# DanielaCourel/smoothed_particle_hydrodynamics

Measured on AMD Instinct MI355X. Metric: Mparticle-steps/sec (whole node), dam-break, higher is better.
Workload: dtype f32

## Files before the change

smoothed_particle_hydrodynamics_amd/csrc/context.h:

```cpp
#pragma once

#include <stdlib.h>
#include <string.h>

#include <memory>
#include <new>
#include <utility>

#include "cell_build.h"
#include "common_kernels.h"
#include "full_kernels.h"
#include "full_tiled.h"
#include "ref_kernels.h"
#include "sample_kernels.h"
#include "surface_kernels.h"
#include "render_kernels.h"
#include "scene_kernels.h"
#include "tracer_kernels.h"
#include "gauge_kernels.h"
#include "slab_kernels.h"
#include "slab_rccl.h"

namespace {

// ... 127 lines not shown
   int cur = 0;

   DevBuf<uint32_t> key;
   DevBuf<uint32_t> slot;
   DevBuf<uint32_t> perm;
   DevBuf<uint32_t> order;
   DevBuf<uint32_t> cell_count;
   DevBuf<uint32_t> cell_start;
   DevBuf<uint32_t> scan_part;
   DevBuf<uint32_t> big_cells;
   int scan_tiles = 0;

   DevBuf<float> rho;
   DevBuf<float4> velB;
   DevBuf<float> auxc;
   DevBuf<float4> acc;
   DevBuf<int32_t> ncount;
   DevBuf<TileDesc> tile_desc;
   DevBuf<uint32_t> nlist;
   DevBuf<uint32_t> nlist_overflow;
   int fast = 0;
   struct {
      int valid = 0;
      int fast = 0;
      float rho0 = 0.0f, stiffness = 0.0f, kernel3 = 0.0f;
   } terms;
   int uniform_mass = 0;
   int use_tiled = 1;
   int prehashed = 0;
   int no_prehash = 0, no_fused_integrate = 0, no_fused_slab = 0;
// ... 269 lines not shown
   CREATE_TRY(dev_alloc(ctx->big_cells, cap / RANK_BIG + 2));
   CREATE_TRY(hipMemsetAsync(ctx->big_cells, 0, sizeof(uint32_t), ctx->stream));
   CREATE_TRY(hipMemsetAsync(ctx->cell_count, 0, cells_padded * sizeof(uint32_t), ctx->stream));
   CREATE_TRY(hipMemsetAsync(ctx->cell_start, 0, cells_padded * sizeof(uint32_t), ctx->stream));
   CREATE_TRY(dev_alloc(ctx->rho, cap));
   CREATE_TRY(dev_alloc(ctx->acc, cap));
   CREATE_TRY(dev_alloc(ctx->ncount, cap));
   CREATE_TRY(hipMemsetAsync(ctx->rho, 0, cap * sizeof(float), ctx->stream));
   CREATE_TRY(hipMemsetAsync(ctx->acc, 0, cap * sizeof(float4), ctx->stream));
   CREATE_TRY(hipMemsetAsync(ctx->ncount, 0, cap * sizeof(int32_t), ctx->stream));
   CREATE_TRY(dev_alloc(ctx->meta, META_COUNT));
   CREATE_TRY(hipMemsetAsync(ctx->meta, 0, META_COUNT * sizeof(int32_t), ctx->stream));
   if (mode == SPH_HIP_MODE_FULL) {
      CREATE_TRY(dev_alloc(ctx->velB, cap));
      CREATE_TRY(dev_alloc(ctx->auxc, cap));
      CREATE_TRY(dev_alloc(ctx->tile_desc, (size_t)div_up(capacity, TILE_THREADS) + 1));
      ctx->list_cap = NLIST_CAP;
      ctx->list_cap_max = NLIST_CAP_MAX;
      if (const char* v = getenv("SPH_HIP_LIST_CAP")) {
         const int c = atoi(v) / 2 * 2;
         if (c > 0) ctx->list_cap = ctx->list_cap_max = c < 2 ? 2 : (c > NLIST_CAP_MAX ? NLIST_CAP_MAX : c);
      }
      ctx->list_blocks = (size_t)div_up(capacity, TILE_THREADS) + 1;
      const size_t nlist_words = ctx->list_blocks * list_rows(ctx->list_cap) * TILE_THREADS;
      CREATE_TRY(dev_alloc(ctx->nlist, nlist_words));
      CREATE_TRY(hipMemsetAsync(ctx->nlist, 0, nlist_words * sizeof(uint32_t), ctx->stream));
      CREATE_TRY(dev_alloc(ctx->nlist_overflow, (size_t)div_up(capacity, TILE_THREADS) + 1));
      if (const char* v = getenv("SPH_HIP_UNTILED")) ctx->use_tiled = (v[0] == '1') ? 0 : 1;
      CREATE_TRY(pinned_alloc(ctx->tile_feedback, TSTAT_COUNT));
      memset(ctx->tile_feedback, 0, TSTAT_COUNT * sizeof(int));
// ... 56 lines not shown
```

smoothed_particle_hydrodynamics_amd/csrc/full_kernels.h:

```cpp
#pragma once

#include "pair_math.h"

struct RowRanges {
   uint32_t s[9], e[9];
};

__device__ __forceinline__ void row_ranges(const CellGrid& g, const uint32_t* __restrict__ cell_start,
                                           int cx, int cy, int cz, RowRanges& r)
{
   const int x0 = cx - 1 < 0 ? 0 : cx - 1;
   const int x1 = cx + 1 >= g.nx ? g.nx - 1 : cx + 1;
#pragma unroll
   for (int k = 0; k < 9; k++) {
      const int z = cz + k / 3 - 1;
      const int y = cy + k % 3 - 1;
      if (z < 0 || z >= g.nz || y < 0 || y >= g.ny) {
         r.s[k] = 0;
         r.e[k] = 0;
      } else {
         const int row = (z * g.ny + y) * g.nx;
         r.s[k] = cell_start[row + x0];
         r.e[k] = cell_start[row + x1 + 1];
      }
   }
}

template <bool UNIT_SCALE, bool FAST = false>
__device__ __forceinline__ void density_untiled(int p, const float4* __restrict__ posm,
                                                const uint32_t* __restrict__ cell_start,
                                                const float4* __restrict__ velp, const CellGrid& g,
                                                const PairConsts& k, float* __restrict__ rho,
                                                float4* __restrict__ velB, float* __restrict__ auxc,
                                                int32_t* __restrict__ ncount)
{
   const float4 pi = posm[p];
   int cx, cy, cz;
   cell_of(g, pi.x, pi.y, pi.z, cx, cy, cz);
   RowRanges r;
   row_ranges(g, cell_start, cx, cy, cz, r);

   float density = 0.0f;
   int count = 0;
#pragma unroll 1
   for (int row = 0; row < 9; row++) {
      const uint32_t s = row == 0 ? r.s[0] : row == 1 ? r.s[1] : row == 2 ? r.s[2] : row == 3 ? r.s[3]
                       : row == 4 ? r.s[4] : row == 5 ? r.s[5] : row == 6 ? r.s[6] : row == 7 ? r.s[7] : r.s[8];
      const uint32_t e = row == 0 ? r.e[0] : row == 1 ? r.e[1] : row == 2 ? r.e[2] : row == 3 ? r.e[3]
                       : row == 4 ? r.e[4] : row == 5 ? r.e[5] : row == 6 ? r.e[6] : row == 7 ? r.e[7] : r.e[8];
// ... 5 lines not shown
         if (d2 < k.h2) {
            {
               float d = sqrtf(d2);
               if (!UNIT_SCALE) d *= k.sim_scale;
               density_accumulate<UNIT_SCALE>(k, pj.w, d, density);
            }
            count++;
         }
      }
   }
   rho[p] = density;
   const float2 bc = FAST ? neighbor_terms_fast(k, density, pi.w) : neighbor_terms(k, density, pi.w);
   const float4 v = velp[p];
   velB[p] = make_float4(v.x, v.y, v.z, FAST ? bc.y : bc.x);
   auxc[p] = FAST ? bc.x : bc.y;
   ncount[p] = count;
}

template <bool FAST>
__global__ void __launch_bounds__(256)
k_neighbor_terms(const float4* __restrict__ posm, const float4* __restrict__ velp,
                 const float* __restrict__ rho, const int32_t* __restrict__ meta, PairConsts k,
                 float4* __restrict__ velB, float* __restrict__ auxc)
{
   const int p = meta[META_SUM_BEGIN] + blockIdx.x * blockDim.x + threadIdx.x;
   if (p >= meta[META_SUM_END]) return;
   const float2 bc = FAST ? neighbor_terms_fast(k, rho[p], posm[p].w) : neighbor_terms(k, rho[p], posm[p].w);
   const float4 v = velp[p];
   velB[p] = make_float4(v.x, v.y, v.z, FAST ? bc.y : bc.x);
   auxc[p] = FAST ? bc.x : bc.y;
}

template <bool UNIT_SCALE, bool FAST>
__global__ void __launch_bounds__(256)
k_full_density(const float4* __restrict__ posm, const uint32_t* __restrict__ cell_start,
               const float4* __restrict__ velp, const int32_t* __restrict__ meta, CellGrid g,
               PairConsts k, float* __restrict__ rho, float4* __restrict__ velB,
               float* __restrict__ auxc, int32_t* __restrict__ ncount)
{
   const int p = meta[META_SUM_BEGIN] + blockIdx.x * blockDim.x + threadIdx.x;
   if (p >= meta[META_SUM_END]) return;
   density_untiled<UNIT_SCALE, FAST>(p, posm, cell_start, velp, g, k, rho, velB, auxc, ncount);
}

template <bool UNIT_SCALE, bool FAST = false>
__device__ __forceinline__ void accel_untiled(int p, const float4* __restrict__ posm,
                                              const float4* __restrict__ velB,
                                              const float* __restrict__ rho,
                                              const float* __restrict__ auxc,
                                              const uint32_t* __restrict__ cell_start,
                                              const CellGrid& g, const PairConsts& k,
                                              float4* __restrict__ acc,
                                              const int32_t* __restrict__ ncount = nullptr)
{
   const float4 pi = posm[p];
   int cx, cy, cz;
   cell_of(g, pi.x, pi.y, pi.z, cx, cy, cz);
// ... 51 lines not shown
```

smoothed_particle_hydrodynamics_amd/csrc/full_tiled.h:

```cpp
#pragma once

#include "launch_policy.h"
#include "common_kernels.h"
#include "full_kernels.h"
#include "neighbor_lists.h"
#include "slab_kernels.h"

#if defined(SPH_ABLATE) && !defined(SPH_DIAGNOSTIC_BUILD)
#error "SPH_ABLATE is for diagnostic builds only: add -DSPH_DIAGNOSTIC_BUILD (tools/build_variant.sh does)"
#endif

#ifdef SPH_TRIPCOUNT
#ifndef SPH_DIAGNOSTIC_BUILD
#error "SPH_TRIPCOUNT is for diagnostic builds only: add -DSPH_DIAGNOSTIC_BUILD"
#endif
enum {
   TRIP_D_WAVES = 0, TRIP_D_CHUNKS_W, TRIP_D_TEST8_W, TRIP_D_TEST8_L, TRIP_D_SLOTS_L, TRIP_D_POPS_W,
   TRIP_D_POPS_L, TRIP_D_POPLOOPS_W, TRIP_D_SUMTRIPS_W, TRIP_D_SUMSLOTS_W, TRIP_D_LISTED_L, TRIP_D_LANES_L,
   TRIP_A_WAVES = 16, TRIP_A_PTRIPS_W, TRIP_A_CNT_L, TRIP_A_VTRIPS_W, TRIP_A_NV_L, TRIP_A_LANES_L,
   TRIP_COUNT = 32
};
__device__ unsigned long long g_trip[TRIP_COUNT];
struct TripCounters {
   unsigned int v[16];
// ... 30 lines not shown
   }
#define PHASE_COUNT(i) if (threadIdx.x == 0 && blockIdx.x < PHASE_WGS) g_phase[(i) >> 4][blockIdx.x][7] = 1u
#else
#define PHASE_BEGIN()
#define PHASE_MARK(i)
#define PHASE_COUNT(i)
#endif

constexpr int TILE_BATCH = 8;
#define DENSITY_TILE_BYTES 12
#define ACCEL_TILE_BYTES 16
constexpr int DENSITY_BLOCKS = 6 * 256 / TILE_THREADS;
constexpr int ACCEL_BLOCKS = TILE_THREADS == 256 ? 5 : 2;
constexpr int APPEND_POPS = 4;
constexpr int VISC_UNROLL = 4;

typedef float __attribute__((ext_vector_type(2))) f32x2;
typedef float __attribute__((ext_vector_type(4))) f32x4;

__device__ __forceinline__ f32x4 lds_read4(const float* base, int i)
{
   return *reinterpret_cast<const f32x4*>(__builtin_assume_aligned(base + i, 16));
}

struct TileDesc {
   int D[9];
   int B[9];
   int total;
   int pad;
};
// ... 96 lines not shown

__device__ __forceinline__ void tile_desc_load(const TileDesc* __restrict__ desc, int wg, TileDesc& sd)
{
   const int tid = threadIdx.x;
   if (tid < (int)(sizeof(TileDesc) / sizeof(int)))
      reinterpret_cast<int*>(&sd)[tid] = reinterpret_cast<const int*>(&desc[wg])[tid];
   __syncthreads();
}

__device__ __forceinline__ int xcd_workgroup(int block, int nblocks)
{
   const int q = nblocks / 8, r = nblocks % 8, x = block % 8;
   return (x < r ? x * (q + 1) : r * (q + 1) + (x - r) * q) + block / 8;
}

__device__ __forceinline__ void tile_load(const float4* __restrict__ posm, const TileDesc& sd,
                                          const TileLds& L)
{
   const int tid = threadIdx.x;
   const int total = sd.total;
   int B[9], D[9];
#pragma unroll
   for (int k = 0; k < 9; k++) {
      B[k] = sd.B[k];
      D[k] = sd.D[k];
   }
#if defined(SPH_ABLATE) && (SPH_ABLATE == 3 || SPH_ABLATE == 5)
   for (int base = 0; base < 0; base += TILE_BATCH * TILE_THREADS) {
#else
   for (int base = 0; base < total; base += TILE_BATCH * TILE_THREADS) {
#endif
      float4 buf[TILE_BATCH];
#pragma unroll
      for (int r = 0; r < TILE_BATCH; r++) {
         const int idx = min(base + tid + r * TILE_THREADS, total - 1);
         int d = D[0];
#pragma unroll
         for (int k = 1; k < 9; k++) d = (idx >= B[k]) ? D[k] : d;
         buf[r] = posm[idx - d];
      }
#pragma unroll
      for (int r = 0; r < TILE_BATCH; r++) {
         const int idx = base + tid + r * TILE_THREADS;
         if (idx < total) {
            L.x[idx] = buf[r].x;
            L.y[idx] = buf[r].y;
            L.z[idx] = buf[r].z;
         }
      }
   }
   __syncthreads();
}


// ... 46 lines not shown
   m = __builtin_amdgcn_alignbit(m, __float_as_uint(dc.y), 31);
   m = __builtin_amdgcn_alignbit(m, __float_as_uint(dc.x), 31);
   m = __builtin_amdgcn_alignbit(m, __float_as_uint(db.y), 31);
   m = __builtin_amdgcn_alignbit(m, __float_as_uint(db.x), 31);
   m = __builtin_amdgcn_alignbit(m, __float_as_uint(da.y), 31);
   m = __builtin_amdgcn_alignbit(m, __float_as_uint(da.x), 31);
   return m;
}

template <bool UNIT_SCALE, bool UNIFORM_MASS, bool WIDE, bool FAST>
__global__ void __launch_bounds__(TILE_THREADS, WIDE ? (DENSITY_BLOCKS < 4 ? DENSITY_BLOCKS : 4) : DENSITY_BLOCKS)
k_full_density_tiled(const float4* __restrict__ posm, const float4* __restrict__ velp,
                     const uint32_t* __restrict__ cell_start, const int32_t* __restrict__ meta,
                     CellGrid g, PairConsts k, float* __restrict__ rho_out,
                     float4* __restrict__ velB_out, float* __restrict__ auxc_out,
                     int32_t* __restrict__ ncount, const TileDesc* __restrict__ desc,
                     uint32_t* __restrict__ nlist, uint32_t* __restrict__ nlist_overflow,
                     int tile_cap, int32_t* __restrict__ tile_stats,
                     const uint32_t* __restrict__ giveup, int* __restrict__ tile_feedback, int list_cap,
                     double* __restrict__ epart_clear, int inline_giveups)
{
   PHASE_BEGIN();
   if (epart_clear && threadIdx.x < 2) epart_clear[2 * blockIdx.x + threadIdx.x] = 0.0;
   __shared__ TileDesc sd;
   __shared__ int list_overflow;
   TileLds L;
   L.x = tile_lds_dynamic;
   L.y = L.x + (tile_cap + TILE_PAD);
   L.z = L.y + (tile_cap + TILE_PAD);
   if (blockIdx.x == 0 && threadIdx.x < TSTAT_NO_LIST) tile_feedback[threadIdx.x] = tile_stats[threadIdx.x];

   const int begin = meta[META_SUM_BEGIN];
   const int end = meta[META_SUM_END];
   const int tid = threadIdx.x;
   if (inline_giveups && (int)blockIdx.x < tile_stats[TSTAT_GIVEUP_DENSITY]) {
      const int gp = begin + (int)giveup[blockIdx.x] * TILE_THREADS + tid;
      if (gp < end)
         density_untiled<UNIT_SCALE, FAST>(gp, posm, cell_start, velp, g, k, rho_out, velB_out,
                                           auxc_out, ncount);
   }
   const int wgs = tile_stats[TSTAT_BLOCKS];
   const int wg = (int)blockIdx.x < wgs ? xcd_workgroup(blockIdx.x, wgs) : (int)blockIdx.x;
   const int p0 = begin + wg * TILE_THREADS;
   if (p0 >= end) return;
   const int p = p0 + tid;
   const bool live = p < end;
   if (tid == 0) list_overflow = 0;
   float4 pi = make_float4(0.f, 0.f, 0.f, 0.f);
   if (live) pi = posm[p];
   tile_desc_load(desc, wg, sd);
   if (sd.total > tile_cap) {
      if (inline_giveups && tid == 0) nlist_overflow[wg] = LISTS_NONE;
      return;
   }
   char* stage_lane = nullptr;
   const int packed = __builtin_amdgcn_readfirstlane(((sd.total + 31) & ~31) + TILE_PAD);
   const bool staged = (tile_cap + TILE_PAD - packed) * (int)DENSITY_TILE_BYTES >= 16 * TILE_THREADS;
   if (staged) {
      L.y = L.x + packed;
      L.z = L.y + packed;
      stage_lane = reinterpret_cast<char*>(L.z + packed) + 16 * tid;
      list_stage_clear(stage_lane);
   }
   RowRanges r;
#pragma unroll
   for (int kk = 0; kk < 9; kk++) r.s[kk] = r.e[kk] = 0;
   if (live) {
#if !(defined(SPH_ABLATE) && (SPH_ABLATE == 4 || SPH_ABLATE == 5))
      int cx, cy, cz;
      cell_of(g, pi.x, pi.y, pi.z, cx, cy, cz);
      row_ranges(g, cell_start, cx, cy, cz, r);
#endif
   }
   PHASE_MARK(0);
   tile_load(posm, sd, L);
   PHASE_MARK(1);
   const int self_t = p + sd.D[4];
   const f32x2 px = {pi.x, pi.x}, py = {pi.y, pi.y}, pz = {pi.z, pi.z};

   const float h2_screen = k.h2_screen;
   TRIP(TripCounters trips; trips.wave(TRIP_D_WAVES, true); trips.lane(TRIP_D_LANES_L, live ? 1u : 0u);)
   int count = 0;
   ListWriter lw(nlist, wg, list_cap, tid, stage_lane);
   uint32_t pos = list_pos_of(0u);
   auto test_and_append = [&](auto staged_c) {
      constexpr bool STAGED = decltype(staged_c)::value;
#pragma unroll
      for (int kk = 0; kk < 9; kk++) {
         const int D = sd.D[kk];
         const uint32_t kbits = ListEntry<WIDE>::tag(kk);
// ... 150 lines not shown
#endif
   }
   if (!overflowed && kept != count) {
      count = kept;
      lw.pad(count, list_cap);
   }
   TRIP(trips.flush(0, 1u << TRIP_D_TEST8_L | 1u << TRIP_D_SLOTS_L | 1u << TRIP_D_POPS_L | 1u << TRIP_D_LISTED_L |
                       1u << TRIP_D_LANES_L);)
   PHASE_MARK(4);
   if (live) {
      rho_out[p] = density;
      const float2 bc = FAST ? neighbor_terms_fast(k, density, pi.w) : neighbor_terms(k, density, pi.w);
      const float4 v = velp[p];
      velB_out[p] = make_float4(v.x, v.y, v.z, FAST ? bc.y : bc.x);
      auxc_out[p] = FAST ? bc.x : bc.y;
      ncount[p] = count;
   }
   PHASE_MARK(5);
   PHASE_COUNT(15);
}

template <bool UNIT_SCALE, bool UNIFORM_MASS, bool WIDE, bool FAST>
__global__ void __launch_bounds__(TILE_THREADS, 4)
k_full_density_chunked(const float4* __restrict__ posm, const float4* __restrict__ velp,
                       const uint32_t* __restrict__ cell_start, const int32_t* __restrict__ meta,
                       CellGrid g, PairConsts k, float* __restrict__ rho_out,
                       float4* __restrict__ velB_out, float* __restrict__ auxc_out,
                       int32_t* __restrict__ ncount, const TileDesc* __restrict__ desc,
                       uint32_t* __restrict__ nlist, uint32_t* __restrict__ nlist_overflow,
                       int tile_cap, int32_t* __restrict__ tile_stats,
                       const uint32_t* __restrict__ giveup, int list_cap)
{
   __shared__ TileDesc sd;
   __shared__ int list_overflow;
   const int tid = threadIdx.x;
   const bool staged = tile_cap >= 1024;
   const int chunk_cap = staged ? tile_cap - 352 : tile_cap;
   TileLds L;
   L.x = tile_lds_dynamic;
   L.y = L.x + (chunk_cap + TILE_PAD);
   L.z = L.y + (chunk_cap + TILE_PAD);
   char* const stage_lane = reinterpret_cast<char*>(L.z + (chunk_cap + TILE_PAD)) + 16 * tid;
   const int begin = meta[META_SUM_BEGIN], end = meta[META_SUM_END];
   const int n_giveup = tile_stats[TSTAT_GIVEUP_DENSITY];
   for (int gi = blockIdx.x; gi < n_giveup; gi += gridDim.x) {
      const int wg = (int)giveup[gi];
      const int p0 = begin + wg * TILE_THREADS;
      const int p = p0 + tid;
      const bool live = p < end;
      __syncthreads();
      if (tid == 0) list_overflow = 0;
      tile_desc_load(desc, wg, sd);
      if (sd.total + TILE_PAD > (1 << ListEntry<WIDE>::TBITS)) {
         if (live) density_untiled<UNIT_SCALE, FAST>(p, posm, cell_start, velp, g, k, rho_out, velB_out, auxc_out, ncount);
         if (tid == 0) nlist_overflow[wg] = LISTS_NONE;
         continue;
      }
      float4 pi = make_float4(0.f, 0.f, 0.f, 0.f);
      RowRanges r;
#pragma unroll
      for (int kk = 0; kk < 9; kk++) r.s[kk] = r.e[kk] = 0;
      if (live) {
         pi = posm[p];
         int cx, cy, cz;
         cell_of(g, pi.x, pi.y, pi.z, cx, cy, cz);
         row_ranges(g, cell_start, cx, cy, cz, r);
      }
      int cxa, cya, cza, cxb, cyb, czb;
      const float4 pa = posm[p0], pb = posm[min(p0 + TILE_THREADS - 1, end - 1)];
// ... 77 lines not shown
                        } else {
                           count++;
                           if (staged) lw.append<true>(pos, ebase + bit);
                           else lw.append<false>(pos, ebase + bit);
                        }
                     }
                  }
               }
            }
         }
      }
      const bool overflowed = lw.finish(pos, count, list_cap, staged, list_overflow);
      lists_publish(overflowed, list_overflow, tile_stats, nlist_overflow, wg);
      if (live) {
         if (overflowed) {
            density_untiled<UNIT_SCALE, FAST>(p, posm, cell_start, velp, g, k, rho_out, velB_out, auxc_out, ncount);
         } else {
            rho_out[p] = density;
            const float2 bc = FAST ? neighbor_terms_fast(k, density, pi.w) : neighbor_terms(k, density, pi.w);
            const float4 v = velp[p];
            velB_out[p] = make_float4(v.x, v.y, v.z, FAST ? bc.y : bc.x);
            auxc_out[p] = FAST ? bc.x : bc.y;
            ncount[p] = count;
         }
      }
   }
}

struct AccelLds {
   TileDesc desc;
};

__device__ __forceinline__ bool accel_part_has(int part, int p0, const int32_t* __restrict__ meta)
{
   if (part == 0) return true;
   const int ob = meta[META_OWN_BEGIN], oe = meta[META_OWN_END];
   const int lo_end = min(meta[META_BND_LO_END], oe);
// ... 193 lines not shown
            } else {
               accel_pair<UNIT_SCALE>(k, s, dx, dy, dz, dd, UNIFORM_MASS ? pi.w : pj[u].w, vj[u].x, vj[u].y,
                                      vj[u].z, vj[u].w, cj[u], in_range);
            }
         }
      }
   }
   if (FAST) accel_fast_finish(k, s);
   return accel_end<UNIT_SCALE>(k, s);
}

template <bool UNIT_SCALE, bool UNIFORM_MASS, bool WIDE, bool FAST>
__global__ void __launch_bounds__(TILE_THREADS, ACCEL_BLOCKS)
k_full_accel_lists(const float4* __restrict__ posm, const float4* __restrict__ velB,
                   const float* __restrict__ rho, const float* __restrict__ auxc,
                   const int32_t* __restrict__ ncount, const uint32_t* __restrict__ cell_start,
                   const int32_t* __restrict__ meta, CellGrid g, PairConsts k,
                   float4* __restrict__ acc, const TileDesc* __restrict__ desc,
                   const uint32_t* __restrict__ nlist, const uint32_t* __restrict__ nlist_overflow,
                   int tile_cap, const int32_t* __restrict__ tile_stats,
                   const uint32_t* __restrict__ giveup, int part, int list_cap,
                   int* __restrict__ tile_feedback, FusedStep fs, int tile_cap_density)
{
   PHASE_BEGIN();
   __shared__ AccelLds L;
   float4* xyzc = reinterpret_cast<float4*>(tile_lds_dynamic);
   constexpr int BATCH = TILE_BATCH;

   const int begin = meta[META_SUM_BEGIN], end = meta[META_SUM_END];
   const int ob = meta[META_OWN_BEGIN], oe = meta[META_OWN_END];
// ... 2 lines not shown
   const int mapped = accel_part_workgroup(part, blockIdx.x, wgs, begin, meta);
   const int wg = mapped < 0 ? 0 : mapped;
   const int p0 = begin + wg * TILE_THREADS;
   if (blockIdx.x == 0 && tid == 0) {
      tile_feedback[TSTAT_NO_LIST] = tile_stats[TSTAT_NO_LIST];
      if (fs.slab && part == 1) {
         if (fs.left) fs.left->header[1] = fs.msg_capacity;
         if (fs.right) fs.right->header[1] = fs.msg_capacity;
      }
   }
   const bool own = mapped >= 0 && !(p0 >= end || p0 + TILE_THREADS <= ob || p0 >= oe) &&
                    accel_part_has(part, p0, meta);
   const uint32_t gave_up = own ? nlist_overflow[wg] : LISTS_NONE;
   int desc_word = 0;
   if (tid < (int)(sizeof(TileDesc) / sizeof(int))) desc_word = reinterpret_cast<const int*>(&desc[wg])[tid];
   if ((int)blockIdx.x < tile_stats[TSTAT_GIVEUP_ACCEL]) {
      const int g0 = begin + (int)giveup[blockIdx.x] * TILE_THREADS;
      const int gp = g0 + tid;
      const bool mine = gp < end && gp >= ob && gp < oe && accel_part_has(part, g0, meta);
      const int gwg = (int)giveup[blockIdx.x];
      const uint32_t glists = nlist_overflow[gwg];
      if (glists != LISTS_NONE) {
         tile_desc_load(desc, gwg, L.desc);
         if (mine) {
            const int gcnt = ncount[gp];
            const ListReader glr(nlist, gwg, list_cap, tid);
            if (glists == LISTS_SOME && gcnt > 0 && glr.no_list())
               accel_untiled<UNIT_SCALE, FAST>(gp, posm, velB, rho, auxc, cell_start, g, k, acc, ncount);
            else
               acc[gp] = accel_from_lists<UNIT_SCALE, UNIFORM_MASS, WIDE, FAST>(gp, gcnt, glr, L.desc, posm, velB,
// ... 4 lines not shown
         accel_untiled<UNIT_SCALE, FAST>(gp, posm, velB, rho, auxc, cell_start, g, k, acc, ncount);
      }
      if (fs.on && accel_part_has(part, g0, meta)) {
         float4 gx = make_float4(0.f, 0.f, 0.f, 0.f), ga = gx;
         if (mine) {
            gx = posm[gp];
            ga = acc[gp];
         }
         fused_integrate<UNIT_SCALE>(fs, k, g, gp, mine, gx, ga, (int)giveup[blockIdx.x]);
      }
   }
   if (gave_up == LISTS_NONE) return;
   if (tid < (int)(sizeof(TileDesc) / sizeof(int))) reinterpret_cast<int*>(&L.desc)[tid] = desc_word;
   __syncthreads();
   PHASE_MARK(16);
   const int total = L.desc.total;
   if (total > tile_cap || total > tile_cap_density) return;
   int B[9], D[9];
#pragma unroll
   for (int kk = 0; kk < 9; kk++) {
      B[kk] = L.desc.B[kk];
      D[kk] = L.desc.D[kk];
   }
   float4 buf[BATCH];
   float cbuf[BATCH];
#if defined(SPH_ABLATE) && SPH_ABLATE == 23
#pragma unroll
   for (int r = 0; r < BATCH; r++) {
      buf[r] = make_float4(0.f, 0.f, 0.f, 0.f);
      cbuf[r] = 0.f;
   }
   const int filled = 0;
#else
#pragma unroll
   for (int r = 0; r < BATCH; r++) {
      const int idx = min(tid + r * TILE_THREADS, total - 1);
      int d = D[0];
#pragma unroll
      for (int kk = 1; kk < 9; kk++) d = (idx >= B[kk]) ? D[kk] : d;
      buf[r] = posm[idx - d];
      cbuf[r] = auxc[idx - d];
   }
   const int filled = total;
#endif

   const int col = tid;
   const int p = p0 + col;
   const bool live = p < end && p >= ob && p < oe;
   float4 pi = make_float4(0.f, 0.f, 0.f, 0.f);
   float4 vi = pi;
   float rho_i = 0.0f;
   int cnt = 0;
   if (live) {
      pi = posm[p];
      vi = velB[p];
      rho_i = rho[p];
      cnt = ncount[p];
   }

   const ListReader lr(nlist, wg, list_cap, col);
   uint32_t entry[LIST_BLOCK_ENTRIES];
   uint4 next_blk = lr.block(0);

#pragma unroll
   for (int r = 0; r < BATCH; r++) {
      const int idx = tid + r * TILE_THREADS;
      if (idx < filled) xyzc[idx] = make_float4(buf[r].x, buf[r].y, buf[r].z, cbuf[r]);
   }

   AccelState s;
   int first_v = 0;
   bool no_list = false;
   float4 vpre[VISC_UNROLL];
   int tpre[VISC_UNROLL], nvp = 0;
   uint32_t ev[VISC_UNROLL];
   if constexpr (FAST) {
      static_assert(VISC_UNROLL == 4, "list_entries_from takes four entries");
      accel_begin(k, s, pi, vi, rho_i);
      first_v = visc_first(cnt, s.visc_scale);
      const int lcnt = cnt <= list_cap ? cnt : 0;
      const int fv = lcnt > 0 ? first_v : 0;
      const int lb = lcnt > 0 ? (lcnt - 1) >> 3 : 0;
      const int fb = fv >> 3;
      const uint4 blk_a = lr.block(fb), blk_b = lr.block(min(fb + 1, lb));
      if (gave_up == LISTS_SOME && cnt > 0) no_list = next_blk.x == NLIST_NO_LIST;
      nvp = no_list ? 0 : lcnt - fv;
      list_entries_from(blk_a, blk_b, (uint32_t)(fv & 7), ev);
   }

   for (int base = BATCH * TILE_THREADS; base < filled; base += BATCH * TILE_THREADS) {
#pragma unroll
      for (int r = 0; r < BATCH; r++) {
         const int idx = min(base + tid + r * TILE_THREADS, filled - 1);
         int d = D[0];
#pragma unroll
         for (int kk = 1; kk < 9; kk++) d = (idx >= B[kk]) ? D[kk] : d;
         buf[r] = posm[idx - d];
         cbuf[r] = auxc[idx - d];
      }
#pragma unroll
      for (int r = 0; r < BATCH; r++) {
         const int idx = base + tid + r * TILE_THREADS;
         if (idx < filled) xyzc[idx] = make_float4(buf[r].x, buf[r].y, buf[r].z, cbuf[r]);
      }
   }
   if constexpr (FAST) {
#pragma unroll
      for (int u = 0; u < VISC_UNROLL; u++) {
         tpre[u] = ListEntry<WIDE>::tile(ev[u]);
         vpre[u] = make_float4(0.f, 0.f, 0.f, 0.f);
         if (u < nvp) vpre[u] = velB[tpre[u] - ListEntry<WIDE>::shift(L.desc, ev[u])];
      }
   }
   __syncthreads();

   PHASE_MARK(17);
   if constexpr (!FAST) accel_begin(k, s, pi, vi, rho_i);
   const bool in_range = accel_operands_in_range(k);
   if constexpr (!FAST) {
      if (gave_up == LISTS_SOME && cnt > 0) no_list = next_blk.x == NLIST_NO_LIST;
   }
   if (no_list) cnt = 0;
#if defined(SPH_ABLATE) && (SPH_ABLATE == 21 || SPH_ABLATE == 23)
   cnt = 0;
#endif
   const int lastb = cnt > 0 ? (cnt - 1) >> 3 : 0;
   if constexpr (FAST) {
      TRIP(TripCounters trips; trips.wave(TRIP_A_WAVES - 16, true); trips.lane(TRIP_A_CNT_L - 16, (unsigned)cnt);
// ... 157 lines not shown
```

smoothed_particle_hydrodynamics_amd/csrc/launch.h:

```cpp
#pragma once

#include <math.h>

#include <type_traits>

#include "context.h"

namespace {

template <class F>
void bind_flags(F&& f) { f(); }
template <class F, class... Rest>
void bind_flags(F&& f, bool flag, Rest... rest)
{
   if (flag) bind_flags([&](auto... later) { f(std::true_type{}, later...); }, rest...);
   else bind_flags([&](auto... later) { f(std::false_type{}, later...); }, rest...);
}

PairConsts pair_consts(const sph_hip_params& p, bool fast)
{
   PairConsts k;
   k.h2 = p.h2;
   static const float screen = getenv("SPH_HIP_TEST_SCREEN") ? (float)atof(getenv("SPH_HIP_TEST_SCREEN"))
                                                             : TEST_SCREEN_FACTOR;
// ... 277 lines not shown
      if (!ctx->chunk_stream) {
         if (hipStreamCreateWithFlags(ctx->chunk_stream.out(), hipStreamNonBlocking) != hipSuccess ||
             event_create(ctx->ev_chunk_fork) != hipSuccess || event_create(ctx->ev_chunk_join) != hipSuccess) {
            (void)hipGetLastError();
            ctx->chunk_stream.reset();
         }
      }
      if (ctx->chunk_stream && hipEventRecord(ctx->ev_chunk_fork, ctx->stream) == hipSuccess &&
          hipStreamWaitEvent(ctx->chunk_stream, ctx->ev_chunk_fork, 0) == hipSuccess)
         side = ctx->chunk_stream;
   }
   bind_flags([&](auto U, auto M, auto W, auto F) {
      if (chunked)
         hipLaunchKernelGGL((k_full_density_chunked<U.value, M.value, W.value, F.value>), dim3(1024),
                            dim3(TILE_THREADS), lds, side, ctx->posm[ctx->cur], ctx->velp[ctx->cur],
                            ctx->cell_start, ctx->meta, ctx->grid, k, ctx->rho, ctx->velB, ctx->auxc,
                            ctx->ncount, ctx->tile_desc, ctx->nlist, ctx->nlist_overflow, cap,
                            ctx->tile_stats, ctx->giveup_density, ctx->list_cap);
      hipLaunchKernelGGL((k_full_density_tiled<U.value, M.value, W.value, F.value>), dim3(blocks),
                         dim3(TILE_THREADS), lds, ctx->stream, ctx->posm[ctx->cur], ctx->velp[ctx->cur],
                         ctx->cell_start, ctx->meta, ctx->grid, k, ctx->rho, ctx->velB, ctx->auxc,
                         ctx->ncount, ctx->tile_desc, ctx->nlist, ctx->nlist_overflow, cap,
                         ctx->tile_stats, ctx->giveup_density, ctx->tile_feedback, ctx->list_cap,
                         epart_clear, chunked ? 0 : 1);
   }, unit, ctx->uniform_mass != 0, ctx->caps.wide != 0, ctx->fast != 0);
   if (side != ctx->stream) {
      if (hipEventRecord(ctx->ev_chunk_join, side) != hipSuccess ||
          hipStreamWaitEvent(ctx->stream, ctx->ev_chunk_join, 0) != hipSuccess) {
         (void)hipGetLastError();
         (void)hipStreamSynchronize(side);
      }
   }
}

void launch_accel_lists(sph_hip_context* ctx, bool unit, int blocks, const PairConsts& k, int part,
                        hipStream_t st, bool fused = false, const SlabFused* slab = nullptr)
// ... 11 lines not shown
      fs.cell_count = ctx->cell_count;
      if (slab) {
         fs.slab = 1;
         fs.zone = slab_zone(ctx);
         fs.left = (SlabMsg*)slab->left;
         fs.right = (SlabMsg*)slab->right;
         fs.msg_capacity = slab->capacity;
         fs.meta = ctx->meta;
      }
   }
   const int cap = ctx->caps.cap_accel;
   const size_t lds = (size_t)(cap + TILE_PAD) * ACCEL_TILE_BYTES;
   bind_flags([&](auto U, auto M, auto W, auto F) {
      if constexpr (M.value || !F.value)
      hipLaunchKernelGGL((k_full_accel_lists<U.value, M.value, W.value, F.value>), dim3(blocks),
                         dim3(TILE_THREADS), lds, st, ctx->posm[ctx->cur], ctx->velB, ctx->rho, ctx->auxc,
                         ctx->ncount, ctx->cell_start, ctx->meta, ctx->grid, k, ctx->acc, ctx->tile_desc,
                         ctx->nlist, ctx->nlist_overflow, cap, ctx->tile_stats, ctx->giveup_accel, part,
                         ctx->list_cap, ctx->tile_feedback, fs, ctx->caps.cap_density);
   }, unit, ctx->uniform_mass != 0 || ctx->fast != 0, ctx->caps.wide != 0, ctx->fast != 0);
}

void note_neighbor_terms(sph_hip_context* ctx, const PairConsts& k)
{
   ctx->terms.valid = 1;
   ctx->terms.fast = ctx->fast;
   ctx->terms.rho0 = k.rho0;
   ctx->terms.stiffness = k.stiffness;
   ctx->terms.kernel3 = k.kernel3;
}

void refresh_neighbor_terms(sph_hip_context* ctx, const PairConsts& k)
{
   const bool same = ctx->terms.valid && ctx->terms.fast == ctx->fast &&
                     memcmp(&ctx->terms.rho0, &k.rho0, sizeof(float)) == 0 &&
                     memcmp(&ctx->terms.stiffness, &k.stiffness, sizeof(float)) == 0 &&
                     memcmp(&ctx->terms.kernel3, &k.kernel3, sizeof(float)) == 0;
   if (same) return;
   bind_flags([&](auto F) {
      hipLaunchKernelGGL((k_neighbor_terms<F.value>), dim3(div_up(ctx->n, 256)), dim3(256), 0, ctx->stream,
                         ctx->posm[ctx->cur], ctx->velp[ctx->cur], ctx->rho, ctx->meta, k, ctx->velB,
                         ctx->auxc);
   }, ctx->fast != 0);
   note_neighbor_terms(ctx, k);
}

int launch_density(sph_hip_context* ctx)
{
   const int n = ctx->n;
   if (n == 0) return SPH_HIP_OK;
   const PairConsts k = pair_consts(ctx->prm, ctx->fast != 0);
   const int blocks = div_up(n, 256);
   if (ctx->mode == SPH_HIP_MODE_REF) {
      hipLaunchKernelGGL(k_ref_density, dim3(blocks), dim3(256), 0, ctx->stream, ctx->posm[0],
                         ctx->nb, ctx->nd, ctx->ncount, n, ctx->prm.examine_count, k, ctx->rho);
   } else {
      const bool unit = unit_scale(ctx->prm);
      if (ctx->use_tiled) {
         launch_density_tiled(ctx, unit, div_up(n, TILE_THREADS), k);
      } else {
         bind_flags([&](auto U, auto F) {
            hipLaunchKernelGGL((k_full_density<U.value, F.value>), dim3(blocks), dim3(256), 0, ctx->stream,
                               ctx->posm[ctx->cur], ctx->cell_start, ctx->velp[ctx->cur], ctx->meta,
                               ctx->grid, k, ctx->rho, ctx->velB, ctx->auxc, ctx->ncount);
         }, unit, ctx->fast != 0);
      }
      note_neighbor_terms(ctx, k);
   }
   SPH_TRY(hipGetLastError());
   return SPH_HIP_OK;
}

int launch_accel(sph_hip_context* ctx, int part = 0, hipStream_t part_stream = nullptr, bool fused = false,
                 const SlabFused* slab = nullptr)
{
   const int n = ctx->n;
   if (n == 0) return SPH_HIP_OK;
   const PairConsts k = pair_consts(ctx->prm, ctx->fast != 0);
   const int blocks = div_up(n, 256);
// ... 292 lines not shown
```

Before: 4775.

## Pack position and aux term into one float4 for accel tile fill

Density kernels now also write a packed float4 of position plus the per-particle aux coefficient. The accel kernel fills its LDS tile from this single array instead of separate posm and auxc gathers. Cell-shift lookup becomes wave-uniform via readfirstlane, falling back to per-lane only when a wave straddles a boundary. The tile-fill loop is restructured into request/store lambdas, with an optional direct global-to-LDS load path. This adds an extra float4 store per particle in density and more device memory, in exchange for fewer, wider loads in accel.

```diff
diff --git a/smoothed_particle_hydrodynamics_amd/csrc/context.h b/smoothed_particle_hydrodynamics_amd/csrc/context.h
--- a/smoothed_particle_hydrodynamics_amd/csrc/context.h
+++ b/smoothed_particle_hydrodynamics_amd/csrc/context.h
@@ -165,6 +165,7 @@
    DevBuf<float> rho;
    DevBuf<float4> velB;
    DevBuf<float> auxc;
+   DevBuf<float4> xyzw_tile;
    DevBuf<float4> acc;
    DevBuf<int32_t> ncount;
    DevBuf<TileDesc> tile_desc;
@@ -464,6 +465,7 @@
    if (mode == SPH_HIP_MODE_FULL) {
       CREATE_TRY(dev_alloc(ctx->velB, cap));
       CREATE_TRY(dev_alloc(ctx->auxc, cap));
+      CREATE_TRY(dev_alloc(ctx->xyzw_tile, cap));
       CREATE_TRY(dev_alloc(ctx->tile_desc, (size_t)div_up(capacity, TILE_THREADS) + 1));
       ctx->list_cap = NLIST_CAP;
       ctx->list_cap_max = NLIST_CAP_MAX;
diff --git a/smoothed_particle_hydrodynamics_amd/csrc/full_kernels.h b/smoothed_particle_hydrodynamics_amd/csrc/full_kernels.h
--- a/smoothed_particle_hydrodynamics_amd/csrc/full_kernels.h
+++ b/smoothed_particle_hydrodynamics_amd/csrc/full_kernels.h
@@ -26,13 +26,18 @@
    }
 }
 
+__device__ __forceinline__ void tile_record_store(float4* __restrict__ xyzw_tile, int p, const float4& pi, float c)
+{
+   xyzw_tile[p] = make_float4(pi.x, pi.y, pi.z, c);
+}
+
 template <bool UNIT_SCALE, bool FAST = false>
 __device__ __forceinline__ void density_untiled(int p, const float4* __restrict__ posm,
                                                 const uint32_t* __restrict__ cell_start,
                                                 const float4* __restrict__ velp, const CellGrid& g,
                                                 const PairConsts& k, float* __restrict__ rho,
                                                 float4* __restrict__ velB, float* __restrict__ auxc,
-                                                int32_t* __restrict__ ncount)
+                                                float4* __restrict__ xyzw_tile, int32_t* __restrict__ ncount)
 {
    const float4 pi = posm[p];
    int cx, cy, cz;
@@ -68,6 +73,7 @@
    const float4 v = velp[p];
    velB[p] = make_float4(v.x, v.y, v.z, FAST ? bc.y : bc.x);
    auxc[p] = FAST ? bc.x : bc.y;
+   tile_record_store(xyzw_tile, p, pi, FAST ? bc.x : bc.y);
    ncount[p] = count;
 }
 
@@ -75,14 +81,16 @@
 __global__ void __launch_bounds__(256)
 k_neighbor_terms(const float4* __restrict__ posm, const float4* __restrict__ velp,
                  const float* __restrict__ rho, const int32_t* __restrict__ meta, PairConsts k,
-                 float4* __restrict__ velB, float* __restrict__ auxc)
+                 float4* __restrict__ velB, float* __restrict__ auxc, float4* __restrict__ xyzw_tile)
 {
    const int p = meta[META_SUM_BEGIN] + blockIdx.x * blockDim.x + threadIdx.x;
    if (p >= meta[META_SUM_END]) return;
-   const float2 bc = FAST ? neighbor_terms_fast(k, rho[p], posm[p].w) : neighbor_terms(k, rho[p], posm[p].w);
+   const float4 pi = posm[p];
+   const float2 bc = FAST ? neighbor_terms_fast(k, rho[p], pi.w) : neighbor_terms(k, rho[p], pi.w);
    const float4 v = velp[p];
    velB[p] = make_float4(v.x, v.y, v.z, FAST ? bc.y : bc.x);
    auxc[p] = FAST ? bc.x : bc.y;
+   tile_record_store(xyzw_tile, p, pi, FAST ? bc.x : bc.y);
 }
 
 template <bool UNIT_SCALE, bool FAST>
@@ -90,11 +98,11 @@
 k_full_density(const float4* __restrict__ posm, const uint32_t* __restrict__ cell_start,
                const float4* __restrict__ velp, const int32_t* __restrict__ meta, CellGrid g,
                PairConsts k, float* __restrict__ rho, float4* __restrict__ velB,
-               float* __restrict__ auxc, int32_t* __restrict__ ncount)
+               float* __restrict__ auxc, float4* __restrict__ xyzw_tile, int32_t* __restrict__ ncount)
 {
    const int p = meta[META_SUM_BEGIN] + blockIdx.x * blockDim.x + threadIdx.x;
    if (p >= meta[META_SUM_END]) return;
-   density_untiled<UNIT_SCALE, FAST>(p, posm, cell_start, velp, g, k, rho, velB, auxc, ncount);
+   density_untiled<UNIT_SCALE, FAST>(p, posm, cell_start, velp, g, k, rho, velB, auxc, xyzw_tile, ncount);
 }
 
 template <bool UNIT_SCALE, bool FAST = false>
diff --git a/smoothed_particle_hydrodynamics_amd/csrc/full_tiled.h b/smoothed_particle_hydrodynamics_amd/csrc/full_tiled.h
--- a/smoothed_particle_hydrodynamics_amd/csrc/full_tiled.h
+++ b/smoothed_particle_hydrodynamics_amd/csrc/full_tiled.h
@@ -68,6 +68,12 @@
 constexpr int ACCEL_BLOCKS = TILE_THREADS == 256 ? 5 : 2;
 constexpr int APPEND_POPS = 4;
 constexpr int VISC_UNROLL = 4;
+#ifndef SPH_ACCEL_FILL
+#define SPH_ACCEL_FILL 1
+#endif
+#ifndef SPH_ACCEL_SHIFT_PER_WAVE
+#define SPH_ACCEL_SHIFT_PER_WAVE 1
+#endif
 
 typedef float __attribute__((ext_vector_type(2))) f32x2;
 typedef float __attribute__((ext_vector_type(4))) f32x4;
@@ -194,17 +200,70 @@
    return (x < r ? x * (q + 1) : r * (q + 1) + (x - r) * q) + block / 8;
 }
 
-__device__ __forceinline__ void tile_load(const float4* __restrict__ posm, const TileDesc& sd,
+struct TileShifts {
+   int E[9], D[9], total;
+};
+
+__device__ __forceinline__ void tile_shifts_load(const TileDesc* __restrict__ desc, int wg, TileShifts& ts)
+{
+   const int* w = reinterpret_cast<const int*>(&desc[__builtin_amdgcn_readfirstlane(wg)]);
+   int B[9];
+#pragma unroll
+   for (int k = 0; k < 9; k++) {
+      ts.D[k] = __builtin_amdgcn_readfirstlane(w[k]);
+      B[k] = __builtin_amdgcn_readfirstlane(w[9 + k]);
+   }
+   ts.total = __builtin_amdgcn_readfirstlane(w[18]);
+   bool border[9];
+   int in_force = ts.D[0];
+#pragma unroll
+   for (int k = 1; k < 9; k++) {
+      const bool taken = k == 8 || B[k + 1] > B[k];
+      border[k] = taken & (ts.D[k] != in_force);
+      in_force = taken ? ts.D[k] : in_force;
+   }
+   int above = 0x7fffffff;
+#pragma unroll
+   for (int k = 8; k >= 1; k--) {
+      above = border[k] ? B[k] : above;
+      ts.E[k] = above;
+   }
+   ts.E[0] = 0;
+}
+
+__device__ __forceinline__ int tile_shift(const TileShifts& ts, int idx, int first, int last)
+{
+   int d = ts.D[0];
+#pragma unroll
+   for (int k = 1; k < 9; k++) d = (first >= ts.E[k]) ? ts.D[k] : d;
+#if !defined(SPH_SHIFT_PER_LANE)
+   int next = 0x7fffffff;
+#pragma unroll
+   for (int k = 8; k >= 1; k--) next = (ts.E[k] > first) ? ts.E[k] : next;
+   if (next <= last)
+#endif
+   {
+      d = ts.D[0];
+#pragma unroll
+      for (int k = 1; k < 9; k++) d = (idx >= ts.E[k]) ? ts.D[k] : d;
+   }
+   return d;
+}
+
+__device__ __forceinline__ int tile_shift_lane(const int (&B)[9], const int (&D)[9], int idx)
+{
+   int d = D[0];
+#pragma unroll
+   for (int k = 1; k < 9; k++) d = (idx >= B[k]) ? D[k] : d;
+   return d;
+}
+
+__device__ __forceinline__ void tile_load(const float4* __restrict__ posm, const TileShifts& ts,
                                           const TileLds& L)
 {
    const int tid = threadIdx.x;
-   const int total = sd.total;
-   int B[9], D[9];
-#pragma unroll
-   for (int k = 0; k < 9; k++) {
-      B[k] = sd.B[k];
-      D[k] = sd.D[k];
-   }
+   const int total = ts.total;
+   const int wave_first = __builtin_amdgcn_readfirstlane(tid) & ~(SPH_WAVE - 1);
 #if defined(SPH_ABLATE) && (SPH_ABLATE == 3 || SPH_ABLATE == 5)
    for (int base = 0; base < 0; base += TILE_BATCH * TILE_THREADS) {
 #else
@@ -214,10 +273,8 @@
 #pragma unroll
       for (int r = 0; r < TILE_BATCH; r++) {
          const int idx = min(base + tid + r * TILE_THREADS, total - 1);
-         int d = D[0];
-#pragma unroll
-         for (int k = 1; k < 9; k++) d = (idx >= B[k]) ? D[k] : d;
-         buf[r] = posm[idx - d];
+         const int w0 = base + wave_first + r * TILE_THREADS;
+         buf[r] = posm[idx - tile_shift(ts, idx, min(w0, total - 1), min(w0 + SPH_WAVE - 1, total - 1))];
       }
 #pragma unroll
       for (int r = 0; r < TILE_BATCH; r++) {
@@ -294,6 +351,7 @@
                      const uint32_t* __restrict__ cell_start, const int32_t* __restrict__ meta,
                      CellGrid g, PairConsts k, float* __restrict__ rho_out,
                      float4* __restrict__ velB_out, float* __restrict__ auxc_out,
+                     float4* __restrict__ xyzw_out,
                      int32_t* __restrict__ ncount, const TileDesc* __restrict__ desc,
                      uint32_t* __restrict__ nlist, uint32_t* __restrict__ nlist_overflow,
                      int tile_cap, int32_t* __restrict__ tile_stats,
@@ -317,7 +375,7 @@
       const int gp = begin + (int)giveup[blockIdx.x] * TILE_THREADS + tid;
       if (gp < end)
          density_untiled<UNIT_SCALE, FAST>(gp, posm, cell_start, velp, g, k, rho_out, velB_out,
-                                           auxc_out, ncount);
+                                           auxc_out, xyzw_out, ncount);
    }
    const int wgs = tile_stats[TSTAT_BLOCKS];
    const int wg = (int)blockIdx.x < wgs ? xcd_workgroup(blockIdx.x, wgs) : (int)blockIdx.x;
@@ -328,6 +386,8 @@
    if (tid == 0) list_overflow = 0;
    float4 pi = make_float4(0.f, 0.f, 0.f, 0.f);
    if (live) pi = posm[p];
+   TileShifts ts;
+   tile_shifts_load(desc, wg, ts);
    tile_desc_load(desc, wg, sd);
    if (sd.total > tile_cap) {
       if (inline_giveups && tid == 0) nlist_overflow[wg] = LISTS_NONE;
@@ -353,7 +413,7 @@
 #endif
    }
    PHASE_MARK(0);
-   tile_load(posm, sd, L);
+   tile_load(posm, ts, L);
    PHASE_MARK(1);
    const int self_t = p + sd.D[4];
    const f32x2 px = {pi.x, pi.x}, py = {pi.y, pi.y}, pz = {pi.z, pi.z};
@@ -534,6 +594,7 @@
       const float4 v = velp[p];
       velB_out[p] = make_float4(v.x, v.y, v.z, FAST ? bc.y : bc.x);
       auxc_out[p] = FAST ? bc.x : bc.y;
+      tile_record_store(xyzw_out, p, pi, FAST ? bc.x : bc.y);
       ncount[p] = count;
    }
    PHASE_MARK(5);
@@ -546,6 +607,7 @@
                        const uint32_t* __restrict__ cell_start, const int32_t* __restrict__ meta,
                        CellGrid g, PairConsts k, float* __restrict__ rho_out,
                        float4* __restrict__ velB_out, float* __restrict__ auxc_out,
+                       float4* __restrict__ xyzw_out,
                        int32_t* __restrict__ ncount, const TileDesc* __restrict__ desc,
                        uint32_t* __restrict__ nlist, uint32_t* __restrict__ nlist_overflow,
                        int tile_cap, int32_t* __restrict__ tile_stats,
@@ -572,7 +634,7 @@
       if (tid == 0) list_overflow = 0;
       tile_desc_load(desc, wg, sd);
       if (sd.total + TILE_PAD > (1 << ListEntry<WIDE>::TBITS)) {
-         if (live) density_untiled<UNIT_SCALE, FAST>(p, posm, cell_start, velp, g, k, rho_out, velB_out, auxc_out, ncount);
+         if (live) density_untiled<UNIT_SCALE, FAST>(p, posm, cell_start, velp, g, k, rho_out, velB_out, auxc_out, xyzw_out, ncount);
          if (tid == 0) nlist_overflow[wg] = LISTS_NONE;
          continue;
       }
@@ -680,13 +742,14 @@
       lists_publish(overflowed, list_overflow, tile_stats, nlist_overflow, wg);
       if (live) {
          if (overflowed) {
-            density_untiled<UNIT_SCALE, FAST>(p, posm, cell_start, velp, g, k, rho_out, velB_out, auxc_out, ncount);
+            density_untiled<UNIT_SCALE, FAST>(p, posm, cell_start, velp, g, k, rho_out, velB_out, auxc_out, xyzw_out, ncount);
          } else {
             rho_out[p] = density;
             const float2 bc = FAST ? neighbor_terms_fast(k, density, pi.w) : neighbor_terms(k, density, pi.w);
             const float4 v = velp[p];
             velB_out[p] = make_float4(v.x, v.y, v.z, FAST ? bc.y : bc.x);
             auxc_out[p] = FAST ? bc.x : bc.y;
+            tile_record_store(xyzw_out, p, pi, FAST ? bc.x : bc.y);
             ncount[p] = count;
          }
       }
@@ -910,6 +973,7 @@
 __global__ void __launch_bounds__(TILE_THREADS, ACCEL_BLOCKS)
 k_full_accel_lists(const float4* __restrict__ posm, const float4* __restrict__ velB,
                    const float* __restrict__ rho, const float* __restrict__ auxc,
+                   const float4* __restrict__ xyzw_tile,
                    const int32_t* __restrict__ ncount, const uint32_t* __restrict__ cell_start,
                    const int32_t* __restrict__ meta, CellGrid g, PairConsts k,
                    float4* __restrict__ acc, const TileDesc* __restrict__ desc,
@@ -942,6 +1006,10 @@
    const uint32_t gave_up = own ? nlist_overflow[wg] : LISTS_NONE;
    int desc_word = 0;
    if (tid < (int)(sizeof(TileDesc) / sizeof(int))) desc_word = reinterpret_cast<const int*>(&desc[wg])[tid];
+#if SPH_ACCEL_SHIFT_PER_WAVE
+   TileShifts ts;
+   tile_shifts_load(desc, wg, ts);
+#endif
    if ((int)blockIdx.x < tile_stats[TSTAT_GIVEUP_ACCEL]) {
       const int g0 = begin + (int)giveup[blockIdx.x] * TILE_THREADS;
       const int gp = g0 + tid;
@@ -976,35 +1044,84 @@
    if (tid < (int)(sizeof(TileDesc) / sizeof(int))) reinterpret_cast<int*>(&L.desc)[tid] = desc_word;
    __syncthreads();
    PHASE_MARK(16);
+#if SPH_ACCEL_SHIFT_PER_WAVE
+   const int total = ts.total;
+#define ACCEL_SHIFT_OF(idx, first, last) tile_shift(ts, idx, first, last)
+#else
    const int total = L.desc.total;
-   if (total > tile_cap || total > tile_cap_density) return;
    int B[9], D[9];
 #pragma unroll
    for (int kk = 0; kk < 9; kk++) {
       B[kk] = L.desc.B[kk];
       D[kk] = L.desc.D[kk];
    }
+#define ACCEL_SHIFT_OF(idx, first, last) tile_shift_lane(B, D, idx)
+#endif
+   if (total > tile_cap || total > tile_cap_density) return;
+   const int wave_first = __builtin_amdgcn_readfirstlane(tid) & ~(SPH_WAVE - 1);
+#if defined(SPH_ABLATE) && SPH_ABLATE == 23
+   const int filled = 0;
+#else
+   const int filled = total;
+#endif
+#if SPH_ACCEL_FILL == 2
+   auto tile_request = [&](int base) {
+#pragma unroll
+      for (int r = 0; r < BATCH; r++) {
+         const int w0 = base + wave_first + r * TILE_THREADS;
+         const int idx = w0 + (tid & (SPH_WAVE - 1));
+         if (idx < filled) {
+            const int d = ACCEL_SHIFT_OF(idx, w0, min(w0 + SPH_WAVE - 1, total - 1));
+            __builtin_amdgcn_global_load_lds(
+               (const __attribute__((address_space(1))) void*)(xyzw_tile + (idx - d)),
+               (__attribute__((address_space(3))) void*)(xyzc + w0), 16, 0, 0);
+         }
+      }
+   };
+   auto tile_store = [&](int) {};
+#else
+#if SPH_ACCEL_FILL == 0
    float4 buf[BATCH];
    float cbuf[BATCH];
+#else
+   f32x4 buf[BATCH];
+#endif
+   auto tile_request = [&](int base) {
+#pragma unroll
+      for (int r = 0; r < BATCH; r++) {
 #if defined(SPH_ABLATE) && SPH_ABLATE == 23
-#pragma unroll
-   for (int r = 0; r < BATCH; r++) {
-      buf[r] = make_float4(0.f, 0.f, 0.f, 0.f);
-      cbuf[r] = 0.f;
-   }
-   const int filled = 0;
-#else
-#pragma unroll
-   for (int r = 0; r < BATCH; r++) {
-      const int idx = min(tid + r * TILE_THREADS, total - 1);
-      int d = D[0];
-#pragma unroll
-      for (int kk = 1; kk < 9; kk++) d = (idx >= B[kk]) ? D[kk] : d;
-      buf[r] = posm[idx - d];
-      cbuf[r] = auxc[idx - d];
-   }
-   const int filled = total;
-#endif
+#if SPH_ACCEL_FILL == 0
+         buf[r] = make_float4(0.f, 0.f, 0.f, 0.f);
+         cbuf[r] = 0.f;
+#else
+         buf[r] = f32x4{0.f, 0.f, 0.f, 0.f};
+#endif
+#else
+         const int idx = min(base + tid + r * TILE_THREADS, total - 1);
+         const int w0 = base + wave_first + r * TILE_THREADS;
+         const int q = idx - ACCEL_SHIFT_OF(idx, min(w0, total - 1), min(w0 + SPH_WAVE - 1, total - 1));
+#if SPH_ACCEL_FILL == 0
+         buf[r] = posm[q];
+         cbuf[r] = auxc[q];
+#else
+         buf[r] = *reinterpret_cast<const f32x4*>(xyzw_tile + q);
+#endif
+#endif
+      }
+   };
+   auto tile_store = [&](int base) {
+#pragma unroll
+      for (int r = 0; r < BATCH; r++) {
+         const int idx = base + tid + r * TILE_THREADS;
+#if SPH_ACCEL_FILL == 0
+         if (idx < filled) xyzc[idx] = make_float4(buf[r].x, buf[r].y, buf[r].z, cbuf[r]);
+#else
+         if (idx < filled) *reinterpret_cast<f32x4*>(xyzc + idx) = buf[r];
+#endif
+      }
+   };
+#endif
+   tile_request(0);
 
    const int col = tid;
    const int p = p0 + col;
@@ -1024,11 +1141,7 @@
    uint32_t entry[LIST_BLOCK_ENTRIES];
    uint4 next_blk = lr.block(0);
 
-#pragma unroll
-   for (int r = 0; r < BATCH; r++) {
-      const int idx = tid + r * TILE_THREADS;
-      if (idx < filled) xyzc[idx] = make_float4(buf[r].x, buf[r].y, buf[r].z, cbuf[r]);
-   }
+   tile_store(0);
 
    AccelState s;
    int first_v = 0;
@@ -1050,30 +1163,29 @@
       list_entries_from(blk_a, blk_b, (uint32_t)(fv & 7), ev);
    }
 
+   auto visc_gathers = [&]() {
+      if constexpr (FAST) {
+#pragma unroll
+         for (int u = 0; u < VISC_UNROLL; u++) {
+            tpre[u] = ListEntry<WIDE>::tile(ev[u]);
+            vpre[u] = make_float4(0.f, 0.f, 0.f, 0.f);
+            if (u < nvp) vpre[u] = velB[tpre[u] - ListEntry<WIDE>::shift(L.desc, ev[u])];
+         }
+      }
+   };
+#ifdef SPH_ACCEL_GATHERS_FIRST
+   visc_gathers();
+#endif
    for (int base = BATCH * TILE_THREADS; base < filled; base += BATCH * TILE_THREADS) {
-#pragma unroll
-      for (int r = 0; r < BATCH; r++) {
-         const int idx = min(base + tid + r * TILE_THREADS, filled - 1);
-         int d = D[0];
-#pragma unroll
-         for (int kk = 1; kk < 9; kk++) d = (idx >= B[kk]) ? D[kk] : d;
-         buf[r] = posm[idx - d];
-         cbuf[r] = auxc[idx - d];
-      }
-#pragma unroll
-      for (int r = 0; r < BATCH; r++) {
-         const int idx = base + tid + r * TILE_THREADS;
-         if (idx < filled) xyzc[idx] = make_float4(buf[r].x, buf[r].y, buf[r].z, cbuf[r]);
-      }
-   }
-   if constexpr (FAST) {
-#pragma unroll
-      for (int u = 0; u < VISC_UNROLL; u++) {
-         tpre[u] = ListEntry<WIDE>::tile(ev[u]);
-         vpre[u] = make_float4(0.f, 0.f, 0.f, 0.f);
-         if (u < nvp) vpre[u] = velB[tpre[u] - ListEntry<WIDE>::shift(L.desc, ev[u])];
-      }
-   }
+      tile_request(base);
+      tile_store(base);
+   }
+#ifndef SPH_ACCEL_GATHERS_FIRST
+   visc_gathers();
+#endif
+#if SPH_ACCEL_FILL == 2
+   asm volatile("s_waitcnt vmcnt(0)" ::: "memory");
+#endif
    __syncthreads();
 
    PHASE_MARK(17);
diff --git a/smoothed_particle_hydrodynamics_amd/csrc/launch.h b/smoothed_particle_hydrodynamics_amd/csrc/launch.h
--- a/smoothed_particle_hydrodynamics_amd/csrc/launch.h
+++ b/smoothed_particle_hydrodynamics_amd/csrc/launch.h
@@ -315,12 +315,12 @@
       if (chunked)
          hipLaunchKernelGGL((k_full_density_chunked<U.value, M.value, W.value, F.value>), dim3(1024),
                             dim3(TILE_THREADS), lds, side, ctx->posm[ctx->cur], ctx->velp[ctx->cur],
-                            ctx->cell_start, ctx->meta, ctx->grid, k, ctx->rho, ctx->velB, ctx->auxc,
+                            ctx->cell_start, ctx->meta, ctx->grid, k, ctx->rho, ctx->velB, ctx->auxc, ctx->xyzw_tile,
                             ctx->ncount, ctx->tile_desc, ctx->nlist, ctx->nlist_overflow, cap,
                             ctx->tile_stats, ctx->giveup_density, ctx->list_cap);
       hipLaunchKernelGGL((k_full_density_tiled<U.value, M.value, W.value, F.value>), dim3(blocks),
                          dim3(TILE_THREADS), lds, ctx->stream, ctx->posm[ctx->cur], ctx->velp[ctx->cur],
-                         ctx->cell_start, ctx->meta, ctx->grid, k, ctx->rho, ctx->velB, ctx->auxc,
+                         ctx->cell_start, ctx->meta, ctx->grid, k, ctx->rho, ctx->velB, ctx->auxc, ctx->xyzw_tile,
                          ctx->ncount, ctx->tile_desc, ctx->nlist, ctx->nlist_overflow, cap,
                          ctx->tile_stats, ctx->giveup_density, ctx->tile_feedback, ctx->list_cap,
                          epart_clear, chunked ? 0 : 1);
@@ -362,7 +362,7 @@
    bind_flags([&](auto U, auto M, auto W, auto F) {
       if constexpr (M.value || !F.value)
       hipLaunchKernelGGL((k_full_accel_lists<U.value, M.value, W.value, F.value>), dim3(blocks),
-                         dim3(TILE_THREADS), lds, st, ctx->posm[ctx->cur], ctx->velB, ctx->rho, ctx->auxc,
+                         dim3(TILE_THREADS), lds, st, ctx->posm[ctx->cur], ctx->velB, ctx->rho, ctx->auxc, ctx->xyzw_tile,
                          ctx->ncount, ctx->cell_start, ctx->meta, ctx->grid, k, ctx->acc, ctx->tile_desc,
                          ctx->nlist, ctx->nlist_overflow, cap, ctx->tile_stats, ctx->giveup_accel, part,
                          ctx->list_cap, ctx->tile_feedback, fs, ctx->caps.cap_density);
@@ -388,7 +388,7 @@
    bind_flags([&](auto F) {
       hipLaunchKernelGGL((k_neighbor_terms<F.value>), dim3(div_up(ctx->n, 256)), dim3(256), 0, ctx->stream,
                          ctx->posm[ctx->cur], ctx->velp[ctx->cur], ctx->rho, ctx->meta, k, ctx->velB,
-                         ctx->auxc);
+                         ctx->auxc, ctx->xyzw_tile);
    }, ctx->fast != 0);
    note_neighbor_terms(ctx, k);
 }
@@ -410,7 +410,7 @@
          bind_flags([&](auto U, auto F) {
             hipLaunchKernelGGL((k_full_density<U.value, F.value>), dim3(blocks), dim3(256), 0, ctx->stream,
                                ctx->posm[ctx->cur], ctx->cell_start, ctx->velp[ctx->cur], ctx->meta,
-                               ctx->grid, k, ctx->rho, ctx->velB, ctx->auxc, ctx->ncount);
+                               ctx->grid, k, ctx->rho, ctx->velB, ctx->auxc, ctx->xyzw_tile, ctx->ncount);
          }, unit, ctx->fast != 0);
       }
       note_neighbor_terms(ctx, k);
```

After: 4810, median of 6. About the same (+0.7%).
